# AHupuJR/REFID

Measured on AMD Instinct MI355X. Metric: interpolated frames/sec (train step) GoPro 256x256 11+1, higher is better.
Workload: dtype f32

## Files before the change

refid_amd/csrc/conv_args.h:

```cpp
#pragma once

struct ConvKArgs {
    const float* inA; const float* inB;
    int ldA, ldB, Ca, Ctot;
    const float* w; const float* bias;
    float* out; int ldO;
    const float* res; int ldR;
    const float* mask; int ldM;
    int N, H, W, Ho, Wo;
    int Cout, CoutPad, coBase;
    int pad, nchunks, tilesX, tilesY;
    float slopePre, slopePost, slopeMask;
    long long wClsStride;
    int vecOK;
    int ncot;
    int bf16;
    int ksplit = 1;
    long long wsStride = 0;
    int gridTiles = 0;
    const float* add2 = nullptr; float* out2 = nullptr; int ldA2 = 0, ldO2 = 0;
    int maskMode = 0;
    int shuffle = 0;
    int patchW = 0, patchRow = 0;
};


size_t refid_wino3x3_workspace_bytes(const ConvKArgs& a, int split_mode);
int refid_launch_wino3x3(const ConvKArgs& a, float* ws, size_t ws_bytes, int split_mode, int tile_hint, hipStream_t st);
int refid_launch_splitk_finish(const ConvKArgs& f, const float* ws, int ldW, long long npix, hipStream_t st);
bool refid_wino6_eligible(const ConvKArgs& a);
size_t refid_wino6_workspace_bytes(const ConvKArgs& a, int split_mode);
int refid_launch_wino6(const ConvKArgs& a, float* ws, size_t ws_bytes, int split_mode, int tile_hint, int terms, hipStream_t st);
bool refid_split3x3_eligible(const ConvKArgs& a);
int refid_launch_split3x3(const ConvKArgs& a, int terms, int mode, int cus, int split_mode, hipStream_t st);
struct PwExtra {
    const float* lnG = nullptr; const float* lnB = nullptr; float lnEps = 0.f; float* lnOut = nullptr; int ldLn = 0;
    const float* pool = nullptr; int poolParts = 0; float invHW = 0.f; int hw = 0; int seC = 0;
    const float* seW1 = nullptr; const float* seB1 = nullptr; const float* seW2 = nullptr; const float* seB2 = nullptr;
    float* seM = nullptr; float* seZ1 = nullptr; float* seS = nullptr;
    float* xsOut = nullptr; int ldXs = 0;
    const float* res2 = nullptr; int ldR2 = 0;
    float* out2 = nullptr; int ldO2 = 0;
};
int refid_launch_pointwise(const ConvKArgs& a, hipStream_t st, const PwExtra* ex = nullptr, int terms = 0);
```

refid_amd/csrc/conv_igemm.hip:

```cpp
#include "common.h"
#include "conv_args.h"

namespace {

template <int KH_, int KW_, int S_, int WM_, int WN_, int MT_, int NT_, int NSUB_, int MODE_>
struct Cfg {
    static constexpr int KH = KH_, KW = KW_, S = S_, WM = WM_, WN = WN_, MT = MT_, NT = NT_;
    static constexpr int NSUB = NSUB_, MODE = MODE_;
    static constexpr int TW = 32;
    static constexpr int TH = WM * MT;
    static constexpr int BN = WN * NT * 32;
    static constexpr int NTAPS = (MODE == 2) ? 4 : KH * KW;
    static constexpr int HH = (MODE == 2) ? TH + 2 : (TH - 1) * S + KH;
    static constexpr int HWD = (MODE == 2) ? TW + 2 : (TW - 1) * S + KW;
    static constexpr int HP = HH * HWD;
    static constexpr int NQ = NSUB * 2;
    static constexpr int KC = NSUB * 8;
    static constexpr int A_TOTAL = HP * NQ;
    static constexpr int B_TOTAL = NTAPS * BN * NQ;
    static constexpr int A_ITEMS = (A_TOTAL + 255) / 256;
    static constexpr int B_ITEMS = (B_TOTAL + 255) / 256;
    static constexpr int LDS_BYTES = (A_TOTAL + B_TOTAL) * 16;
    static_assert(WM * WN == 4, "4 waves per workgroup");
    static_assert(256 % NQ == 0, "thread -> channel-quad mapping must be static");
// ... 371 lines not shown
    a.Ca = d->c_a; a.Ctot = d->c_a + d->c_b;
    a.N = d->n; a.H = d->h; a.W = d->w; a.Ho = d->ho; a.Wo = d->wo;
    a.Cout = d->cout; a.CoutPad = d->cout_pad; a.coBase = d->co_base;
    a.vecOK = 1;
    if (d->algo == 1) return refid_wino3x3_workspace_bytes(a, d->split_k);
    if (d->algo == 5) return refid_wino6_workspace_bytes(a, d->split_k);
    if (d->algo != 0 && d->algo != 2) return 0;
    const bool bf = d->algo == 2;
    const int bn = refid_conv_bn(d->kh, d->kw, d->stride, d->mode, d->cout);
    switch (family_of(d->kh, d->kw, d->stride, d->mode)) {
        case F_4x4s2: return igemm_ws_bytes<C4S2_64>(a, 1, d->split_k, bf);
        case F_downDgrad: return bn == 64 ? igemm_ws_bytes<CD_64>(a, 4, d->split_k, bf) : igemm_ws_bytes<CD_128>(a, 4, d->split_k, bf);
        default: return 0;
    }
}

extern "C" int refid_conv2d(const refid_conv_desc* d, void* stream) {
    hipStream_t st = reinterpret_cast<hipStream_t>(stream);
    REFID_CHECK(d != nullptr, "conv2d: null descriptor");
    const Family f = family_of(d->kh, d->kw, d->stride, d->mode);
    REFID_CHECK(f != F_none, "conv2d: unsupported geometry k=%dx%d stride=%d mode=%d", d->kh, d->kw,
                d->stride, d->mode);
    REFID_CHECK(d->in_a && d->w_packed && d->out, "conv2d: null tensor pointer");
    REFID_CHECK(d->c_a > 0 && d->c_a % 4 == 0 && d->c_b % 4 == 0 && d->c_b >= 0,
                "conv2d: channel counts must be multiples of 4 (c_a=%d c_b=%d)", d->c_a, d->c_b);
    REFID_CHECK(d->ld_a % 4 == 0 && (d->c_b == 0 || d->ld_b % 4 == 0),
                "conv2d: pixel pitches must be multiples of 4 floats");
    REFID_CHECK(d->c_b == 0 || d->in_b != nullptr, "conv2d: c_b > 0 but in_b is null");
    REFID_CHECK(d->n > 0 && d->h > 0 && d->w > 0 && d->ho > 0 && d->wo > 0 && d->cout > 0,
                "conv2d: empty problem (n=%d h=%d w=%d ho=%d wo=%d cout=%d)", d->n, d->h, d->w, d->ho,
                d->wo, d->cout);
    REFID_CHECK(d->pw == nullptr || d->algo == 3, "conv2d: pw fusions belong to the pointwise tile (algo 3)");
    REFID_CHECK(d->algo == 0 || d->algo == 2 || ((d->algo == 1 || d->algo == 5) && f == F_3x3) || (d->algo == 3 && (f == F_1x1 || f == F_convT || f == F_2x2s2)) ||
                    (d->algo == 4 && (f == F_3x3 || f == F_4x4s2 || f == F_downDgrad)),
                "conv2d: algo %d does not fit this geometry (1 / 5 = 3x3 stride 1, 3 = 1x1 and ConvTranspose2d(2,2), 4 = 3x3 stride 1 / 4x4 stride 2 and "
                "its input gradient)", d->algo);
    REFID_CHECK(d->algo != 2 || d->c_b == 0 || d->c_a % 8 == 0, "conv2d: bf16 tile needs c_a %% 8 == 0 for two sources");
    const int bn = refid_conv_bn(d->kh, d->kw, d->stride, d->mode, d->cout);
    REFID_CHECK(d->co_base >= 0 && d->co_base + d->cout <= d->cout_pad,
                "conv2d: rows [%d, %d) exceed the packed weight's %d rows", d->co_base, d->co_base + d->cout,
                d->cout_pad);
    if (d->mode == 0) {
        const int eh = (d->h + 2 * d->pad - d->kh) / d->stride + 1;
        const int ew = (d->w + 2 * d->pad - d->kw) / d->stride + 1;
        REFID_CHECK(eh == d->ho && ew == d->wo, "conv2d: output size %dx%d does not match geometry (%dx%d)",
                    d->ho, d->wo, eh, ew);
    } else {
        REFID_CHECK(d->ho == d->h && d->wo == d->w, "conv2d: mode %d needs ho,wo == h,w", d->mode);
        REFID_CHECK(d->mode != 1 || d->cout % 4 == 0, "conv2d: mode 1 needs cout = 4*Co");
    }
    ConvKArgs a;
    a.inA = d->in_a; a.inB = d->in_b; a.ldA = d->ld_a; a.ldB = d->ld_b;
    a.Ca = d->c_a; a.Ctot = d->c_a + d->c_b;
    a.w = d->w_packed; a.bias = d->bias;
    a.out = d->out; a.ldO = d->ld_out;
    a.res = d->res; a.ldR = d->ld_res;
    a.mask = d->mask; a.ldM = d->ld_mask;
    a.add2 = d->add2; a.ldA2 = d->ld_add2; a.out2 = d->out2; a.ldO2 = d->ld_out2;
    a.maskMode = d->mask_mode;
    REFID_CHECK(d->mask_mode == 0 || (d->mask_mode == 1 && d->algo == 3 && d->mask != nullptr),
                "conv2d: mask_mode 1 (GELU derivative) belongs to the pointwise tile (algo 3) and needs a mask tensor");
    REFID_CHECK(d->out2 == nullptr || (d->add2 != nullptr && (d->algo != 3 || d->pw == nullptr)),
                "conv2d: out2 needs add2 (and, on the pointwise tile, no fusions)");
    a.N = d->n; a.H = d->h; a.W = d->w; a.Ho = d->ho; a.Wo = d->wo;
    a.Cout = d->cout; a.CoutPad = d->cout_pad; a.coBase = d->co_base;
    a.pad = d->pad; a.nchunks = 0; a.tilesX = a.tilesY = 0;
    a.slopePre = d->slope_pre; a.slopePost = d->slope_post; a.slopeMask = d->slope_mask;
    auto al16 = [](const void* p) { return (reinterpret_cast<uintptr_t>(p) & 15) == 0; };
    a.vecOK = al16(d->out) && d->ld_out % 4 == 0 && (!d->res || (al16(d->res) && d->ld_res % 4 == 0)) &&
// ... 21 lines not shown
            REFID_CHECK((long long)d->n * d->h * d->w * d->ld_a * 4 < 0x7fffffffLL, "conv2d: tensor too large for the pointwise tile's 32-bit offsets");
            return refid_launch_pointwise(a, st, nullptr, 0);
        }
        REFID_CHECK(d->c_b == 0 || d->c_a % 8 == 0, "conv2d: pointwise tile needs c_a %% 8 == 0 for two sources");
        const long long lim = 0x7fffffffLL;
        REFID_CHECK((long long)d->n * d->h * d->w * d->ld_a * 4 < lim &&
                        (d->c_b == 0 || (long long)d->n * d->h * d->w * d->ld_b * 4 < lim),
                    "conv2d: tensor too large for the pointwise tile's 32-bit offsets (use algo 0)");
        if (d->pw != nullptr) {
            const refid_pw_extras* x = d->pw;
            PwExtra e;
            e.lnG = x->ln_gamma; e.lnB = x->ln_beta; e.lnEps = x->ln_eps; e.lnOut = x->ln_out; e.ldLn = x->ld_ln_out;
            e.pool = x->pool; e.poolParts = x->pool_parts; e.invHW = x->inv_hw; e.hw = x->hw; e.seC = x->se_c;
            e.seW1 = x->se_w1; e.seB1 = x->se_b1; e.seW2 = x->se_w2; e.seB2 = x->se_b2;
            e.seM = x->se_m; e.seZ1 = x->se_z1; e.seS = x->se_s;
            e.xsOut = x->xs_out; e.ldXs = x->ld_xs_out;
            e.res2 = x->res2; e.ldR2 = x->ld_res2;
            e.out2 = x->out2; e.ldO2 = x->ld_out2;
            auto al = [](const void* q, int ld) { return (reinterpret_cast<uintptr_t>(q) & 15) == 0 && ld % 4 == 0; };
            REFID_CHECK((!e.lnOut || al(e.lnOut, e.ldLn)) && (!e.xsOut || al(e.xsOut, e.ldXs)) && (!e.res2 || al(e.res2, e.ldR2)) &&
                            (!e.out2 || al(e.out2, e.ldO2)) && (!e.lnG || (al(e.lnG, 4) && al(e.lnB, 4))),
                        "conv2d: pointwise fusion tensors must be 16-byte aligned with pitches that are multiples of 4");
            return refid_launch_pointwise(a, st, &e, d->mfma_terms);
        }
        return refid_launch_pointwise(a, st, nullptr, d->mfma_terms);
    }
    if (d->algo == 4) {
        static int cus = 0;
        if (cus == 0) cus = refid_device_cu_count();
        REFID_CHECK(d->pad == 1, "conv2d: the split tile's geometries all have pad 1");
        return refid_launch_split3x3(a, d->mfma_terms ? d->mfma_terms : 6, f == F_3x3 ? 0 : (f == F_4x4s2 ? 1 : 2),
                                     cus > 0 ? cus : 256, d->split_k, st);
    }
    if (d->algo == 5) return refid_launch_wino6(a, d->ws, d->ws_bytes, d->split_k, d->wino_tile, d->mfma_terms, st);
    if (d->algo == 1) {
        REFID_CHECK(d->c_b == 0 || d->c_a % 8 == 0, "conv2d: Winograd tile needs c_a %% 8 == 0 for two sources");
        const long long lim = 0x7fffffffLL;
        REFID_CHECK((long long)d->n * d->h * d->w * d->ld_a * 4 < lim &&
                        (d->c_b == 0 || (long long)d->n * d->h * d->w * d->ld_b * 4 < lim),
                    "conv2d: tensor too large for the Winograd tile's 32-bit offsets (use algo 0)");
        return refid_launch_wino3x3(a, d->ws, d->ws_bytes, d->split_k, d->wino_tile, st);
    }
    switch (f) {
        case F_3x3:
            if (bn == 32) return launch<C3_32>(a, 1, st);
            if (bn == 64) return launch<C3_64>(a, 1, st);
            return launch<C3_128>(a, 1, st);
        case F_5x5: return launch<C5_32>(a, 1, st);
        case F_1x1:
            if (bn == 32) return launch<C1_32>(a, 1, st);
            if (bn == 64) return launch<C1_64>(a, 1, st);
            return launch<C1_128>(a, 1, st);
        case F_4x4s2: return launch<C4S2_64>(a, 1, st, SplitArgs{d->ws, d->ws_bytes, d->split_k});
        case F_2x2s2: return bn == 64 ? launch<C2S2_64>(a, 1, st) : launch<C2S2_128>(a, 1, st);
        case F_convT: return bn == 64 ? launch<CT_64>(a, 1, st) : launch<CT_128>(a, 1, st);
        case F_downDgrad: {
            const SplitArgs sp{d->ws, d->ws_bytes, d->split_k};
            return bn == 64 ? launch<CD_64>(a, 4, st, sp) : launch<CD_128>(a, 4, st, sp);
        }
        default: break;
    }
    refid_set_error("conv2d: no tile for this geometry");
    return 1;
}
```

refid_amd/engine.py:

```python
import os
from collections import OrderedDict

import torch

from . import ops
from ._lib import RefidHipError


def param_shapes(img_chn, ev_chn=2, out_chn=3, base=32, num_residual_blocks=2, num_block=1, num_encoders=3):
    b = base
    sh = OrderedDict()

    def conv(name, co, ci, k, bias=True):
        sh[name + ".weight"] = (co, ci, k, k)
        if bias:
            sh[name + ".bias"] = (co,)

    conv("head.conv2d", b, ev_chn, 5)
    enc_in = [b * 2 ** i for i in range(num_encoders)]
    enc_out = [b * 2 ** (i + 1) for i in range(num_encoders)]

    def evr(prefix, ci, co, fuse, atten):
        conv(prefix + ".conv.conv2d", co, ci, 3)
        if atten:
# ... 100 lines not shown
def use_pipeline(b, h, w):
    return PIPELINE if isinstance(PIPELINE, bool) else b * h * w <= PIPELINE_MAX_PIX
PACK_BATCH = os.environ.get("REFID_PACK_BATCH", "1") != "0"
LAZY_FALLBACK_PACKS = os.environ.get("REFID_LAZY_PACKS", "1") != "0"
CONVT_PW = os.environ.get("REFID_CONVT_PW", "1") != "0"
CONVT_PWS = os.environ.get("REFID_CONVT_PWS", "1") != "0"
ROWS_DEFER = os.environ.get("REFID_ROWS_DEFER", "0") != "0"
FINISH_BATCH = os.environ.get("REFID_FINISH_BATCH", "1") != "0"
FUSE_SUMS = os.environ.get("REFID_FUSE_SUMS", "1") != "0"
LINEAR_SPLIT = os.environ.get("REFID_LINEAR_SPLIT", "1") != "0"


class _SideStreams:
    def __init__(self):
        self._s = {}

    def get(self, device):
        if device.type != "cuda":
            return None
        s = self._s.get(device.index)
        if s is None:
            s = self._s[device.index] = torch.cuda.Stream(device=device)
        return s


DEC_STREAM = _SideStreams()
LV_STREAMS = (_SideStreams(), _SideStreams(), _SideStreams())
WINO6 = os.environ.get("REFID_WINO6", "1") != "0"
_WF16 = os.environ.get("REFID_WINO_F16", "1")
WINO_F16_FWD = _WF16 in ("1", "fwd")
WINO_F16_DGRAD = _WF16 in ("1", "dgrad")
WINO6_MIN_CO = int(os.environ.get("REFID_WINO6_MIN_CO", "32"))
WINO6_THIN = os.environ.get("REFID_WINO6_THIN", "1") != "0"
DOWN_SPLIT = int(os.environ.get("REFID_DOWN_SPLIT", "6"))
WGRAD_WINO_MIN_CO = int(os.environ.get("REFID_WGRAD_WINO_MIN_CO", "32"))
_WG_ENV = os.environ.get("REFID_WGRAD_GROUP")
WGRAD_GROUP = max(1, min(24, int(_WG_ENV))) if _WG_ENV else 24
WGRAD_KEEP_BYTES_PER_PIXEL_STEP = 4900
PWS_WGRAD = os.environ.get("REFID_PWS_WGRAD", "1") != "0"
WGRAD_F4 = os.environ.get("REFID_WGRAD_F4", "1") != "0"
WGRAD_F4_MIN_HW = int(os.environ.get("REFID_WGRAD_F4_MIN_HW", "16"))
WGRAD_DOWN_F4 = os.environ.get("REFID_WGRAD_DOWN_F4", "1") != "0"


def wgrad_group_cap(n, pixels, device, free_bytes=None):
    if n <= 1 or pixels <= 0:
        return n
    if free_bytes is None:
        if torch.device(device).type != "cuda":
            return n
        free_bytes = torch.cuda.mem_get_info(device)[0] + (torch.cuda.memory_reserved(device) - torch.cuda.memory_allocated(device))
    per_step = pixels * WGRAD_KEEP_BYTES_PER_PIXEL_STEP
    return max(1, min(n, int(free_bytes // 2 // per_step)))


FILL_MIN_WG = int(os.environ.get("REFID_FILL_MIN_WG", "256"))


def _fills_gpu(n, ho, wo, cout, classes):
    if ops.WINO_SPLIT != 2:
        n = 8
    return n * -(-ho // 4) * -(-wo // 32) * -(-cout // 64) * classes >= FILL_MIN_WG


_LIM4 = (2 ** 31 - 1) // 4

# ... 134 lines not shown
        if wd6 is not None and wd6.nbytes() >= 2 ** 31 - 1:
            wd6 = None
        terms = 1 if bf16 else (3 if compute_dtype == "bf16x3" else 0)
        sf_pad = sd_pad = 0
        if terms and kind == "conv" and k == 3 and ci % 8 == 0 and co >= 16:
            self.split = terms
            planes = {1: 1, 3: 2}[terms]
            sf_bn = ops.conv_bn(3, 3, 1, 0, co)
            sf_pad = -(-co // sf_bn) * sf_bn
            if not (fp16 and wp6 is not None):
                wps = _Packing("wps", "split", (ops.ROLE_FWD, sf_bn, 3, 3, co, ci, planes))
            if need_dgrad and co % 8 == 0 and (not (fp16 and wd6 is not None) or (ci == 2 * co and co < WINO6_MIN_CO)):
                sd_bn = self.d_bn if self.d_algo != 1 else ops.conv_bn(3, 3, 1, 0, min(ci, 128))
                if ci == 2 * co:
                    sd_bn = ops.conv_bn(3, 3, 1, 0, co)
                sd_pad = -(-ci // sd_bn) * sd_bn
                wds = _Packing("wds", "split", (ops.ROLE_DGRAD, sd_bn, 3, 3, co, ci, planes))
        if kind == "down" and ci % 8 == 0 and co % 8 == 0 and (terms or DOWN_SPLIT):
            self.split = terms = terms or DOWN_SPLIT
            planes = {1: 1, 3: 2, 6: 3, ops.TERMS_F16X3: 2}[terms]
            f16 = terms == ops.TERMS_F16X3
            if not bf16:
                sf_bn = ops.conv_bn(4, 4, 2, 0, co)
                sf_pad = -(-co // sf_bn) * sf_bn
                wps = _Packing("wps", "split", (ops.ROLE_FWD, sf_bn, 4, 4, co, ci, planes), f16)
            if need_dgrad:
                sd_bn = ops.conv_bn(4, 4, 2, 2, ci)
                sd_pad = -(-ci // sd_bn) * sd_bn
                wds = _Packing("wds", "split", (ops.ROLE_DOWN_DGRAD, sd_bn, 4, 4, co, ci, planes), f16)
        self.wp_lazy = wp.lazy = LAZY_FALLBACK_PACKS and wp6 is not None and (self.f_algo == 1 or fp16)
        self.wd_lazy = LAZY_FALLBACK_PACKS and wd6 is not None and (self.d_algo == 1 or fp16)
        if wd is not None:
            wd.lazy = self.wd_lazy
        self.packings = [p for p in (wp, wd, wp6, wd6, wps, wds) if p is not None]
        self._lazy = {p.attr: p for p in self.packings if p.lazy}
        self.wd = self.wp6 = self.wd6 = self.wps = self.wds = None
        for p in self.packings:
            setattr(self, p.attr, p.alloc(self.w.device))
        self.b_eff = self.b
        if self.scale is not None and self.has_bias:
            self.b_eff = torch.empty_like(self.b)
        kh, kw, st, md = f_geo
        self._f_split = self._f_wino6 = self._d_split = self._d_wino6 = self._d_plain = None
        if wps is not None:
            self._f_split = ("wps", dict(kh=kh, kw=kw, stride=st, pad=1, mode=0, cout_pad=sf_pad, algo=4, terms=self.split), True, False)
        if wp6 is not None and (self.split == 0 or fp16):
            self._f_wino6 = ("wp6", dict(kh=3, kw=3, stride=1, pad=1, mode=0, cout_pad=-(-self.f_rows // 64) * 64, algo=5,
                                     terms=wp6.flag), True, False)
        self._f_plain = ("wp", dict(kh=kh, kw=kw, stride=st, pad=self.pad, mode=md, cout_pad=self.f_pad, algo=self.f_algo),
                         self.f_algo != 3, True)
        if need_dgrad:
            kh, kw, st, md = d_geo
            if wds is not None:
                self._d_split = ("wds", dict(kh=kh, kw=kw, stride=st, pad=1, mode=md, cout_pad=sd_pad, algo=4, terms=self.split), True, False)
            if wd6 is not None and (self.split == 0 or fp16):
                self._d_wino6 = ("wd6", dict(kh=3, kw=3, stride=1, pad=1, mode=0, cout_pad=-(-self.d_rows // 64) * 64, algo=5,
                                         terms=wd6.flag), True, False)
            self._d_plain = ("wd", dict(kh=kh, kw=kw, stride=st, pad=d_padding, mode=md, cout_pad=self.d_pad, algo=self.d_algo),
                             self.d_algo != 3 or kind == "convT", self.d_algo == 3 and kind == "conv")
        self.wslab = None
        self.w_calls = 0
        self.w_last = None
        self.w_pend = []
        self.w_algo, self.w_bias = 0, True
        self.w_group = 1

    def plan_repack(self, plan):
        for p in self.packings:
            if not p.lazy:
                p.plan(self, plan)
        if self.scale is not None and self.has_bias:
            plan.add_mul_vec(self.b, self.scale, self.b_eff)

    def _packed(self, attr):
        p = self._lazy.get(attr)
        if p is not None and p.epoch != self.arena.pack_epoch:
            p.pack(self)
        return getattr(self, attr)

    def pack_fallbacks(self):
        for attr in self._lazy:
            self._packed(attr)

    def repack(self):
        for p in self.packings:
            p.pack(self)
        if self.scale is not None and self.has_bias:
            ops.mul_vec(self.b, self.scale, out=self.b_eff)

    def _fwd_route(self, n, ho, wo, a, b, pw):
        r = self._f_split
        if r is not None and (self.split > 1 or b is None) and a.shape[3] % 8 == 0 and pw is None and \
                (self.kind == "conv" or (b is None and _fills_gpu(n, ho, wo, self.co, 1))):
            return r
        r = self._f_wino6
        if r is not None and (b is None or a.shape[3] % 16 == 0):
            return r
        return self._f_plain

    def fwd(self, a, b=None, res=None, slope_pre=1.0, slope_post=1.0, out=None, pw=None, bias=True, plus=None):
        n, h, w, _ = a.shape
        bv = self.b_eff if bias else None
        if self.kind == "conv":
            ho, wo, oc = h, w, self.co
        elif self.kind == "down":
            ho, wo, oc = h // 2, w // 2, self.co
        else:
            ho, wo, oc = 2 * h, 2 * w, self.co
        if out is None:
            out = torch.empty((n, ho, wo, _pad4(oc)), dtype=torch.float32, device=a.device)
            if _pad4(oc) != oc:
                out.zero_()
                out = out[..., :oc]
        o2 = torch.empty_like(out) if plus is not None else None
        parts = ((a, b, res, out),)
        if n * a.stride(0) >= _LIM4 or n * out.stride(0) >= _LIM4 or (b is not None and n * b.stride(0) >= _LIM4):
            if pw is not None:
                raise RefidHipError(f"{self.name}: fused pointwise extras cannot be issued in sub-batches (tensor >= 2 GiB)")
            parts = _sub_batches(n, a, b, res, out)
        for a_i, b_i, res_i, out_i in parts:
            attr, geo, fused, takes_pw = self._fwd_route(a_i.shape[0], ho, wo, a_i, b_i, pw)
            fused = fused and plus is not None and len(parts) == 1
            extra = dict(add2=plus, out2=o2) if fused else {}
            if takes_pw:
                extra["pw"] = pw
            ops.conv2d(a_i, self._packed(attr), out_i, cout=self.f_rows, in_b=b_i, bias=bv, res=res_i, slope_pre=slope_pre,
                       slope_post=slope_post, **geo, **extra)
        if plus is None:
            return out
        if not fused:
            ops.add(out, plus, out=o2)
        return out, o2

    def can_fwd_from(self):
        return self.kind == "conv" and self.k == 1 and self.f_algo == 3 and not self.bf16

    def fwd_from(self, a, k_base):
        if not self.can_fwd_from() or k_base % self.f_kc or a.shape[3] % self.f_kc:
            raise RefidHipError(f"{self.name}: fwd_from needs the fp32 pointwise tile and chunk-aligned channel blocks")
        n, h, w, _ = a.shape
        out = torch.empty((n, h, w, self.co), dtype=torch.float32, device=a.device)
        ops.conv2d(a, self.wp[(k_base // self.f_kc) * self.f_pad * self.f_kc:], out, kh=1, kw=1, stride=1, pad=0, mode=0,
                   cout=self.f_rows, cout_pad=self.f_pad, bias=self.b_eff, algo=3)
        return out

    def _dgrad_route(self, g, cnt):
        r = self._d_wino6
        if self.fp16 and r is not None and cnt >= WINO6_MIN_CO:
            return r
        r = self._d_split
        if r is not None and (self.kind == "conv" or _fills_gpu(g.shape[0], g.shape[1], g.shape[2], cnt, 4)):
            return r
        r = self._d_wino6
        if r is not None and cnt >= WINO6_MIN_CO:
            return r
        return self._d_plain

    def gelu_mask_ok(self, g, rows=None):
        return self.wd is not None and self._dgrad_route(g, rows[1] if rows is not None else self.d_rows)[3]

    def dgrad(self, g, rows=None, res=None, mask=None, slope_mask=1.0, out=None, plus=None, gelu_mask=False):
        if self.wd is None:
            raise RefidHipError(f"{self.name}: dgrad weights were not requested")
        base, cnt = rows if rows is not None else (0, self.d_rows)
        n, h, w, _ = g.shape
        if self.kind == "conv":
            ho, wo = h, w
        elif self.kind == "down":
            ho, wo = 2 * h, 2 * w
        else:
            ho, wo = h // 2, w // 2
        if out is None:
            out = torch.empty((n, ho, wo, cnt), dtype=torch.float32, device=g.device)
        o2 = torch.empty_like(out) if plus is not None else None
        parts = ((g, res, mask, out),)
        if n * g.stride(0) >= _LIM4 or n * out.stride(0) >= _LIM4:
            parts = _sub_batches(n, g, res, mask, out)
        for g_i, res_i, mask_i, out_i in parts:
            attr, geo, fused, gelu_ok = self._dgrad_route(g_i, cnt)
# ... 710 lines not shown
                    if g_Sb[i] is None:
                        g_Sb[i] = L.fuse.dgrad(g_f, rows=(C, C))
                    else:
                        L.fuse.dgrad(g_f, rows=(C, C), res=g_Sb[i], out=g_Sb[i])
                g_s = L.fuse.dgrad(g_f, rows=(0, C), res=g_hf[i])
                g_o = self._evr_first_bwd(L, g_s, st, g_hf, g_xb, g_e, t, B, c["ip_f"], g_skip, True, keep if lin else None)

        if lin:
            self.pred.wgrad(g4sum, head, bias=False)
            g_xb[NL - 1] = ops.sum_n(keep["gb0"])
            for i, L in enumerate(self.enc_f):
                gsum = ops.sum_n(keep["gf"][i])
                if L.zero_s is None:
                    L.fuse.wgrad(gsum, Sb[i], bias=False, i_base=L.C)
                else:
                    L.fuse.wgrad(gsum, L.zero_s, Sb[i], bias=False)
                g_Sb[i] = L.fuse.dgrad(gsum, rows=(L.C, L.C))
            for i in range(2, NL):
                self._lin_level2_tail(self.enc_f[i], keep["gu"][i], xb, g_xb, first=g_xb[i - 1] is None)
            g_xb[0] = ops.sum_n(keep["gy"])
        self._egaca_img_bwd(self.enc_f[1].att, xb[0], g_xb[0], c["ip_f"])
        finish_wgrads(self.early_ops)
        self._egaca_fold_back(self.enc_f[1].att)
        return dict(c=c, B=B, g_xb=g_xb, g_Sb=g_Sb, g_e=g_e, g_head=g_head)

    def backward_late(self, state):
        c, B, g_xb, g_Sb, g_e, g_head = (state[k] for k in ("c", "B", "g_xb", "g_Sb", "g_e", "g_head"))
        xb, head, e_all = c["xb"], c["head"], c["e_all"]
        if ROWS_DEFER:
            ops.rows_sum_defer()
        NL = self.NL
        g_hb = [None] * NL
        lin = c["lin"]
        keep = dict(gy=[], gu={i: [] for i in range(2, NL)})
        for t, sts in reversed(c["steps_b"]):
            g_o = None
            for i in range(NL - 1, -1, -1):
                L, st = self.enc_b[i], sts[i]
                carry = g_hb[i] if g_hb[i] is not None else g_Sb[i]
                if i == NL - 1:
                    g_s = carry
                else:
                    L.down.wgrad(g_o, st["s"])
                    g_s = L.down.dgrad(g_o, res=carry)
                g_o = self._evr_first_bwd(L, g_s, st, g_hb, g_xb, g_e, t, B, c["ip_b"], None, False, keep if lin else None)
        if lin:
            for i in range(2, NL):
                self._lin_level2_tail(self.enc_b[i], keep["gu"][i], xb, g_xb, first=False)
            ops.sum_n([g_xb[0]] + keep["gy"], out=g_xb[0])

        self._egaca_img_bwd(self.enc_b[1].att, xb[0], g_xb[0], c["ip_b"])
        gz_e = ops.act_bwd(g_e, e_all, 0.2, out=g_e)
        self.head_ev.wgrad(gz_e, c["ev_in"])
        g = g_xb[NL - 1]
        for i in range(NL - 1, -1, -1):
            E = self.img[i]
            gin, c1, c2, sm = c["img_saved"][i]
            E["down"].wgrad(g, sm)
            g_sm = E["down"].dgrad(g)
            E["identity"].wgrad(g_sm, gin)
            gz2 = ops.act_bwd(g_sm, c2, 0.2)
            E["conv_2"].wgrad(gz2, c1)
            g_c1 = E["conv_2"].dgrad(gz2, mask=c1, slope_mask=0.2)
            E["conv_1"].wgrad(g_c1, gin)
            acc = g_xb[i - 1] if i > 0 else g_head
            t1 = E["identity"].dgrad(g_sm, res=acc)
            if i > 0:
                g = E["conv_1"].dgrad(g_c1, res=t1)
            else:
                g = E["conv_1"].dgrad(g_c1, res=t1, mask=head, slope_mask=0.2)
        self.head_img.wgrad(g, c["x_in"])
        finish_wgrads(self.all_ops)
        self._egaca_fold_back(self.enc_b[1].att)

    def _lin_level2_tail(self, L, gu, xb, g_xb, first):
        k = L.level - 1
        gsum = ops.sum_n(gu)
        L.conv.wgrad(gsum, xb[k], bias=False)
        if first:
            g_xb[k] = L.conv.dgrad(gsum)
        else:
            L.conv.dgrad(gsum, res=g_xb[k], out=g_xb[k])

    def _evr_first_bwd(self, L, g_s, st, g_h, g_xb, g_e, t, B, ip, g_skip, first_writer, keep=None):
        i = L.level
        lin = keep is not None
        if i == 1:
            g_u, g_h[i] = self._trunk_bwd(L.trunk, g_s, st)
            g_in = self._egaca_bwd(L.att, g_u, None if lin else g_xb[0], ip, st, keep["gy"] if lin else None)
            if g_skip is not None:
                g_in = ops.add(g_in, g_skip[0], out=g_in)
            return g_in
        g_u, g_h[i] = self._trunk_bwd(L.trunk, g_s, st, mask_u=st["u"], slope_u=0.04)
        L.conv.wgrad(g_u, st["src"])
        if i >= 2:
            if lin:
                keep["gu"][i].append(g_u)
                return L.conv.dgrad(g_u, res=g_skip[i - 1] if g_skip is not None else None)
            g_a2 = L.conv.dgrad(g_u)
            ops.add(g_xb[i - 1], g_a2, out=g_xb[i - 1])
            if g_skip is not None:
                g_a2 = ops.add(g_a2, g_skip[i - 1], out=g_a2)
            return g_a2
        sl = g_e[t * B:(t + 1) * B]
        if first_writer:
            L.conv.dgrad(g_u, out=sl)
        else:
            L.conv.dgrad(g_u, res=sl, out=sl)
        return None
```

refid_amd/ops.py:

```python
import ctypes as C
import os

import torch

from . import _lib
from ._lib import ConvDesc, WgradDesc, check, lib

ROLE_FWD, ROLE_DGRAD, ROLE_CONVT, ROLE_CONVT_DGRAD, ROLE_DOWN_DGRAD, ROLE_WINO_FWD, ROLE_WINO_DGRAD, ROLE_CONVT_DGRAD_PW = range(8)


WINO_SPLIT = {"0": 0, "s": 1}.get(os.environ.get("REFID_SPLITK", os.environ.get("REFID_WINO_SPLITK", "auto"))[:1], 2)

WINO_TILE = int(os.environ.get("REFID_WINO_TILE", "0"))

PROFILE = None


def _stream():
    return C.c_void_p(torch.cuda.current_stream().cuda_stream)


_REQUIRE_CUDA = True


# ... 204 lines not shown
    d.slope_pre, d.slope_post, d.slope_mask = slope_pre, slope_post, slope_mask
    d.mask_mode = mask_mode
    d.algo = algo
    d.wino_tile = WINO_TILE
    if WINO_SPLIT and algo in (0, 1, 2, 4, 5):
        d.split_k = WINO_SPLIT
        need = lib().refid_conv_workspace_bytes(C.byref(d))
        if need:
            ws = _workspace(need, in_a.device, "conv")
            d.ws, d.ws_bytes = ws.data_ptr(), ws.numel() * 4
    if PROFILE is None:
        check(lib().refid_conv2d(C.byref(d), _stream()), "refid_conv2d")
        return out
    e0, e1 = torch.cuda.Event(enable_timing=True), torch.cuda.Event(enable_timing=True)
    e0.record()
    check(lib().refid_conv2d(C.byref(d), _stream()), "refid_conv2d")
    e1.record()
    taps = {0: kh * kw, 1: 1, 2: 16}[mode]
    flops = 2.0 * d.n * d.ho * d.wo * cout * (d.c_a + d.c_b) * taps
    name = "conv_igemm_kernel<" + lib().refid_conv_tile_name(kh, kw, stride, mode, cout).decode() + \
        (", true> [bf16 operands]" if algo == 2 else ">")
    if algo == 1:
        name = "conv_wino_kernel<1, 2>" if cout <= 32 else "conv_wino_kernel<2, 1>"
    if algo == 5:
        name = "conv_wino6_kernel<2>" if cout > 32 else "conv_wino6_kernel<1>"
        if terms == 3:
            name = name[:-1] + ", true>"
        if terms == 1:
            name = name[:-1] + ", true, fp16x1>"
    if algo == 4:
        name = "conv_split_kernel<%s>" % ("3, fp16" if terms == TERMS_F16X3 else (terms or 6))
    if algo == 3:
        name = "conv_pw_kernel<1, 8>" if cout <= 32 else ("conv_pw_kernel<2, 4, six>" if terms == 6 else "conv_pw_kernel<2, 4>")
    opix = d.n * out.shape[1] * out.shape[2]
    nbytes = 4.0 * (d.n * d.h * d.w * (d.c_a + d.c_b) + opix * out.shape[3] * (1 + (res is not None) + (mask is not None))
                    + cout * (d.c_a + d.c_b) * taps)
    if out2 is not None:
        nbytes += 8.0 * opix * out.shape[3]
    if pw is not None:
        for k in ("ln_out", "xs_out", "out2", "res2"):
            if pw.get(k) is not None:
                nbytes += 4.0 * pw[k].numel()
    PROFILE.append((name, flops, e0, e1,
                    (d.n, d.h, d.w, d.c_a, d.c_b, cout, int(res is not None), int(mask is not None), int(bias is not None)),
                    nbytes))
    return out


DESC_CACHE = os.environ.get("REFID_DESC_CACHE", "0") == "1"
_DESC_CACHE = {}
_DESC_PTRS = ("in_a", "in_b", "w_packed", "bias", "out", "res", "mask", "add2", "out2")


def _sig(t):
    return None if t is None else (t.shape, t.stride())


def _conv2d_cached(in_a, w_packed, out, kh, kw, stride, pad, mode, cout, cout_pad, co_base, in_b, bias, res, mask,
                   slope_pre, slope_post, slope_mask, algo, terms, add2, out2, mask_mode):
    global lib, DESC_CACHE
    key = (kh, kw, stride, pad, mode, cout, cout_pad, co_base, slope_pre, slope_post, slope_mask, algo, terms, mask_mode,
           WINO_TILE, WINO_SPLIT, _sig(in_a), _sig(in_b), _sig(out), _sig(res), _sig(mask), _sig(add2), _sig(out2),
           bias is not None, in_a.dtype, out.dtype, in_a.device)
    ent = _DESC_CACHE.get(key)
    if ent is None:
        real, seen = lib(), []
# ... 593 lines not shown
```

Before: 515.3.

## Add thin-channel conv kernels for input and output ends, fold head mask into dgrad

Adds a persistent, double-buffered MFMA kernel for convolutions with 4 stored input channels (3x3/5x5), with weights held in registers and halos staged in LDS as channel planes. Also adds an optional direct-FMA kernel for at most 4 output channels, and folds the head's leaky-ReLU backward mask into the last dgrad epilogue so a separate act_bwd pass is skipped. These target the first and last layers, which the generic implicit-GEMM tile wastes work on because it pads channels to 8 or 32. The thin-input forward route and the mask fold are on by default; the dgrad and prediction routes are behind environment flags.

New measurement: 518.4 (median of 6 runs). About the same (+0.6%).

```diff
diff --git a/refid_amd/csrc/conv_args.h b/refid_amd/csrc/conv_args.h
--- a/refid_amd/csrc/conv_args.h
+++ b/refid_amd/csrc/conv_args.h
@@ -43,3 +43,5 @@
     float* out2 = nullptr; int ldO2 = 0;
 };
 int refid_launch_pointwise(const ConvKArgs& a, hipStream_t st, const PwExtra* ex = nullptr, int terms = 0);
+int refid_launch_thin_in(const ConvKArgs& a, int kh, int kw, int stride, int mode, int pairs, hipStream_t st);
+int refid_launch_thin_out(const ConvKArgs& a, int kh, int kw, int stride, int mode, hipStream_t st);
diff --git a/refid_amd/csrc/conv_igemm.hip b/refid_amd/csrc/conv_igemm.hip
--- a/refid_amd/csrc/conv_igemm.hip
+++ b/refid_amd/csrc/conv_igemm.hip
@@ -427,9 +427,10 @@
                 d->wo, d->cout);
     REFID_CHECK(d->pw == nullptr || d->algo == 3, "conv2d: pw fusions belong to the pointwise tile (algo 3)");
     REFID_CHECK(d->algo == 0 || d->algo == 2 || ((d->algo == 1 || d->algo == 5) && f == F_3x3) || (d->algo == 3 && (f == F_1x1 || f == F_convT || f == F_2x2s2)) ||
-                    (d->algo == 4 && (f == F_3x3 || f == F_4x4s2 || f == F_downDgrad)),
-                "conv2d: algo %d does not fit this geometry (1 / 5 = 3x3 stride 1, 3 = 1x1 and ConvTranspose2d(2,2), 4 = 3x3 stride 1 / 4x4 stride 2 and "
-                "its input gradient)", d->algo);
+                    (d->algo == 4 && (f == F_3x3 || f == F_4x4s2 || f == F_downDgrad)) || (d->algo == 6 && (f == F_3x3 || f == F_5x5)) ||
+                    (d->algo == 7 && f == F_3x3),
+                "conv2d: algo %d does not fit this geometry (1 / 5 / 7 = 3x3 stride 1, 3 = 1x1 and ConvTranspose2d(2,2), 4 = 3x3 stride 1 / 4x4 stride 2 and "
+                "its input gradient, 6 = 3x3 / 5x5 stride 1)", d->algo);
     REFID_CHECK(d->algo != 2 || d->c_b == 0 || d->c_a % 8 == 0, "conv2d: bf16 tile needs c_a %% 8 == 0 for two sources");
     const int bn = refid_conv_bn(d->kh, d->kw, d->stride, d->mode, d->cout);
     REFID_CHECK(d->co_base >= 0 && d->co_base + d->cout <= d->cout_pad,
@@ -517,6 +518,8 @@
         return refid_launch_split3x3(a, d->mfma_terms ? d->mfma_terms : 6, f == F_3x3 ? 0 : (f == F_4x4s2 ? 1 : 2),
                                      cus > 0 ? cus : 256, d->split_k, st);
     }
+    if (d->algo == 6) return refid_launch_thin_in(a, d->kh, d->kw, d->stride, d->mode, d->mfma_terms, st);
+    if (d->algo == 7) return refid_launch_thin_out(a, d->kh, d->kw, d->stride, d->mode, st);
     if (d->algo == 5) return refid_launch_wino6(a, d->ws, d->ws_bytes, d->split_k, d->wino_tile, d->mfma_terms, st);
     if (d->algo == 1) {
         REFID_CHECK(d->c_b == 0 || d->c_a % 8 == 0, "conv2d: Winograd tile needs c_a %% 8 == 0 for two sources");
diff --git a/refid_amd/csrc/conv_thin.hip b/refid_amd/csrc/conv_thin.hip
--- /dev/null
+++ b/refid_amd/csrc/conv_thin.hip
@@ -0,0 +1,288 @@
+#include "common.h"
+#include "conv_args.h"
+
+namespace {
+
+__device__ __forceinline__ void thin_epilogue(const ConvKArgs& a, f32x4 v, int j0, long long op, bool vec) {
+    const int ch = j0;
+    f32x4 bv = {0.f, 0.f, 0.f, 0.f};
+    if (a.bias) {
+        const float* bp = a.bias + a.coBase + j0;
+        if (vec) bv = *reinterpret_cast<const f32x4*>(bp);
+        else
+#pragma unroll
+            for (int k = 0; k < 4; ++k) if (j0 + k < a.Cout) bv[k] = bp[k];
+    }
+#pragma unroll
+    for (int k = 0; k < 4; ++k) v[k] = lrelu(v[k] + bv[k], a.slopePre);
+    if (vec) {
+        if (a.res) v += *reinterpret_cast<const f32x4*>(a.res + op * a.ldR + ch);
+#pragma unroll
+        for (int k = 0; k < 4; ++k) v[k] = lrelu(v[k], a.slopePost);
+        if (a.mask) {
+            const f32x4 mv = *reinterpret_cast<const f32x4*>(a.mask + op * a.ldM + ch);
+#pragma unroll
+            for (int k = 0; k < 4; ++k) v[k] *= (mv[k] > 0.f) ? 1.f : a.slopeMask;
+        }
+        *reinterpret_cast<f32x4*>(a.out + op * a.ldO + ch) = v;
+        if (a.out2)
+            *reinterpret_cast<f32x4*>(a.out2 + op * a.ldO2 + ch) = v + *reinterpret_cast<const f32x4*>(a.add2 + op * a.ldA2 + ch);
+    } else {
+#pragma unroll
+        for (int k = 0; k < 4; ++k) {
+            if (j0 + k >= a.Cout) break;
+            float t = v[k];
+            if (a.res) t += a.res[op * a.ldR + ch + k];
+            t = lrelu(t, a.slopePost);
+            if (a.mask) t *= (a.mask[op * a.ldM + ch + k] > 0.f) ? 1.f : a.slopeMask;
+            a.out[op * a.ldO + ch + k] = t;
+            if (a.out2) a.out2[op * a.ldO2 + ch + k] = t + a.add2[op * a.ldA2 + ch + k];
+        }
+    }
+}
+
+template <int K, int NP>
+struct ThinIn {
+    static constexpr int TH = 4, TW = 32;
+    static constexpr int HH = TH + K - 1, HWD = TW + K - 1, HP = HH * HWD;
+    static constexpr int PLANE = HP + ((32 - HP % 64) + 64) % 64;
+    static constexpr int NCH = 2 * NP;
+    static constexpr int ITEMS = (HP + 255) / 256;
+    static constexpr int BUF = NCH * PLANE;
+};
+
+template <int K, int NP>
+__global__ __launch_bounds__(256) void conv_thin_in_kernel(const ConvKArgs a) {
+    using C = ThinIn<K, NP>;
+    __shared__ float sX[2 * C::BUF];
+
+    const int tid = threadIdx.x;
+    const int lane = tid & 63, wave = tid >> 6;
+    const int li = lane & 31, kh = lane >> 5;
+
+    float wr[K * K][NP];
+    {
+        const bool rowOK = li < a.Cout && a.coBase + li < a.CoutPad;
+#pragma unroll
+        for (int t = 0; t < K * K; ++t)
+#pragma unroll
+            for (int p = 0; p < NP; ++p)
+                wr[t][p] = rowOK ? a.w[((long long)t * a.CoutPad + a.coBase + li) * 8 + 2 * p + kh] : 0.f;
+    }
+
+    const float bv = (a.bias && li < a.Cout) ? a.bias[a.coBase + li] : 0.f;
+
+    const int tilesPerImg = a.tilesX * a.tilesY;
+    const int ntiles = tilesPerImg * a.N;
+    f32x4 ra[C::ITEMS];
+
+    auto load_halo = [&](int tile) {
+        const int n = tile / tilesPerImg;
+        const int r = tile - n * tilesPerImg;
+        const int ty = r / a.tilesX, tx = r - ty * a.tilesX;
+        const int iy0 = ty * C::TH - a.pad, ix0 = tx * C::TW - a.pad;
+#pragma unroll
+        for (int it = 0; it < C::ITEMS; ++it) {
+            const int hp = tid + it * 256;
+            const int hy = hp / C::HWD, hx = hp - hy * C::HWD;
+            const int iy = iy0 + hy, ix = ix0 + hx;
+            f32x4 v = {0.f, 0.f, 0.f, 0.f};
+            if (hp < C::HP && iy >= 0 && iy < a.H && ix >= 0 && ix < a.W)
+                v = *reinterpret_cast<const f32x4*>(a.inA + ((long long)(n * a.H + iy) * a.W + ix) * a.ldA);
+            ra[it] = v;
+        }
+    };
+    auto store_halo = [&](float* buf) {
+#pragma unroll
+        for (int it = 0; it < C::ITEMS; ++it) {
+            const int hp = tid + it * 256;
+            if (hp < C::HP) {
+#pragma unroll
+                for (int c = 0; c < C::NCH; ++c) buf[c * C::PLANE + hp] = ra[it][c];
+            }
+        }
+    };
+
+    int tile = blockIdx.x;
+    if (tile >= ntiles) return;
+    load_halo(tile);
+    store_halo(sX);
+    __syncthreads();
+
+    int cur = 0;
+    for (; tile < ntiles; tile += gridDim.x) {
+        const int next = tile + gridDim.x;
+        const bool more = next < ntiles;
+        if (more) load_halo(next);
+
+        const float* pX = sX + cur * C::BUF + kh * C::PLANE + wave * C::HWD + li;
+        f32x16 acc;
+#pragma unroll
+        for (int r = 0; r < 16; ++r) acc[r] = 0.f;
+#pragma unroll
+        for (int t = 0; t < K * K; ++t) {
+            const int toff = (t / K) * C::HWD + (t % K);
+#pragma unroll
+            for (int p = 0; p < NP; ++p)
+                acc = __builtin_amdgcn_mfma_f32_32x32x2f32(pX[2 * p * C::PLANE + toff], wr[t][p], acc, 0, 0, 0);
+        }
+
+        const int n = tile / tilesPerImg;
+        const int rt = tile - n * tilesPerImg;
+        const int ty = rt / a.tilesX, tx = rt - ty * a.tilesX;
+        const int oy = ty * C::TH + wave;
+        if (oy < a.Ho && li < a.Cout) {
+            const long long op0 = (long long)(n * a.Ho + oy) * a.Wo + tx * C::TW;
+            const int wleft = a.Wo - tx * C::TW;
+#pragma unroll
+            for (int r = 0; r < 16; ++r) {
+                const int px = 8 * (r >> 2) + 4 * kh + (r & 3);
+                if (px >= wleft) continue;
+                const long long op = op0 + px;
+                float t = lrelu(acc[r] + bv, a.slopePre);
+                if (a.res) t += a.res[op * a.ldR + li];
+                t = lrelu(t, a.slopePost);
+                if (a.mask) t *= (a.mask[op * a.ldM + li] > 0.f) ? 1.f : a.slopeMask;
+                a.out[op * a.ldO + li] = t;
+                if (a.out2) a.out2[op * a.ldO2 + li] = t + a.add2[op * a.ldA2 + li];
+            }
+        }
+
+        if (more) store_halo(sX + (cur ^ 1) * C::BUF);
+        __syncthreads();
+        cur ^= 1;
+    }
+}
+
+template <int K, int NP>
+int launch_thin_in(const ConvKArgs& ka, int cus, hipStream_t st) {
+    using C = ThinIn<K, NP>;
+    ConvKArgs a = ka;
+    a.tilesX = cdiv(a.Wo, C::TW);
+    a.tilesY = cdiv(a.Ho, C::TH);
+    const long long ntiles = (long long)a.tilesX * a.tilesY * a.N;
+    REFID_CHECK(ntiles < 0x7fffffffLL, "conv2d: too many output tiles for the thin-input tile (algo 6)");
+    long long walk = (ntiles + 16LL * cus - 1) / (16LL * cus);
+    if (walk < 2) walk = 2;
+    const int grid = (int)((ntiles + walk - 1) / walk);
+    hipLaunchKernelGGL((conv_thin_in_kernel<K, NP>), dim3(grid), dim3(256), 0, st, a);
+    REFID_LAUNCH_CHECK("conv_thin_in");
+    return 0;
+}
+
+struct ThinOut {
+    static constexpr int TH = 4, TW = 32, NT = TH * TW;
+    static constexpr int HH = TH + 2, HWD = TW + 2, HP = HH * HWD;
+    static constexpr int NQ = 8;
+    static constexpr int ITEMS = (HP * NQ + NT - 1) / NT;
+};
+
+template <int NCO>
+__global__ __launch_bounds__(ThinOut::NT) void conv_thin_out_kernel(const ConvKArgs a) {
+    using C = ThinOut;
+    __shared__ f32x4 sX[C::NQ * C::HP];
+
+    const int tid = threadIdx.x;
+    int bt = blockIdx.x;
+    const int tx = bt % a.tilesX; bt /= a.tilesX;
+    const int ty = bt % a.tilesY;
+    const int n = bt / a.tilesY;
+    const int iy0 = ty * C::TH - 1, ix0 = tx * C::TW - 1;
+    const int nq = a.Ctot >> 2;
+
+    f32x4 ra[C::ITEMS];
+#pragma unroll
+    for (int it = 0; it < C::ITEMS; ++it) {
+        const int e = tid + it * C::NT;
+        const int q = e % C::NQ, hp = e / C::NQ;
+        const int hy = hp / C::HWD, hx = hp - hy * C::HWD;
+        const int iy = iy0 + hy, ix = ix0 + hx;
+        f32x4 v = {0.f, 0.f, 0.f, 0.f};
+        if (hp < C::HP && q < nq && iy >= 0 && iy < a.H && ix >= 0 && ix < a.W)
+            v = *reinterpret_cast<const f32x4*>(a.inA + ((long long)(n * a.H + iy) * a.W + ix) * a.ldA + 4 * q);
+        ra[it] = v;
+    }
+#pragma unroll
+    for (int it = 0; it < C::ITEMS; ++it) {
+        const int e = tid + it * C::NT;
+        const int q = e % C::NQ, hp = e / C::NQ;
+        if (hp < C::HP) sX[q * C::HP + hp] = ra[it];
+    }
+    __syncthreads();
+
+    const int py = tid >> 5, px = tid & 31;
+    float acc[NCO];
+#pragma unroll
+    for (int co = 0; co < NCO; ++co) acc[co] = 0.f;
+    const float* wrow = a.w + (long long)a.coBase * 8;
+    const int tapStride = a.CoutPad * 8;
+    for (int q = 0; q < nq; ++q) {
+        const float* wq = wrow + (long long)(q >> 1) * 9 * tapStride + (q & 1) * 4;
+        const f32x4* xq = sX + q * C::HP + py * C::HWD + px;
+#pragma unroll
+        for (int t = 0; t < 9; ++t) {
+            const f32x4 x = xq[(t / 3) * C::HWD + (t % 3)];
+#pragma unroll
+            for (int co = 0; co < NCO; ++co) {
+                const f32x4 w = *reinterpret_cast<const f32x4*>(wq + t * tapStride + co * 8);
+#pragma unroll
+                for (int k = 0; k < 4; ++k) acc[co] = __builtin_fmaf(x[k], w[k], acc[co]);
+            }
+        }
+    }
+
+    const int oy = ty * C::TH + py, ox = tx * C::TW + px;
+    if (oy < a.Ho && ox < a.Wo) {
+        const long long op = (long long)(n * a.Ho + oy) * a.Wo + ox;
+        f32x4 v = {0.f, 0.f, 0.f, 0.f};
+#pragma unroll
+        for (int co = 0; co < NCO; ++co) v[co] = acc[co];
+        thin_epilogue(a, v, 0, op, a.vecOK && a.Cout == 4);
+    }
+}
+
+template <int NCO>
+int launch_thin_out(const ConvKArgs& ka, hipStream_t st) {
+    using C = ThinOut;
+    ConvKArgs a = ka;
+    a.tilesX = cdiv(a.Wo, C::TW);
+    a.tilesY = cdiv(a.Ho, C::TH);
+    const long long ntiles = (long long)a.tilesX * a.tilesY * a.N;
+    REFID_CHECK(ntiles < 0x7fffffffLL, "conv2d: too many output tiles for the thin-output tile (algo 7)");
+    hipLaunchKernelGGL((conv_thin_out_kernel<NCO>), dim3((int)ntiles), dim3(C::NT), 0, st, a);
+    REFID_LAUNCH_CHECK("conv_thin_out");
+    return 0;
+}
+
+}
+
+int refid_launch_thin_in(const ConvKArgs& a, int kh, int kw, int stride, int mode, int pairs, hipStream_t st) {
+    REFID_CHECK(stride == 1 && mode == 0, "conv2d: the thin-input tile (algo 6) is stride 1, mode 0 (stride=%d mode=%d)", stride, mode);
+    REFID_CHECK(kh == kw && (kh == 3 || kh == 5), "conv2d: the thin-input tile (algo 6) is 3x3 or 5x5 (kh=%d kw=%d)", kh, kw);
+    REFID_CHECK(a.Ca == 4 && a.Ctot == 4, "conv2d: the thin-input tile (algo 6) takes one source of c_a = 4 stored input channels "
+                "(c_a=%d c_b=%d)", a.Ca, a.Ctot - a.Ca);
+    REFID_CHECK(a.Cout <= 32, "conv2d: the thin-input tile (algo 6) writes at most 32 output channels (cout=%d)", a.Cout);
+    REFID_CHECK(pairs == 0 || pairs == 1 || pairs == 2, "conv2d: algo 6 takes mfma_terms = 1 (input channels 0-1 only) or 0 / 2 (all four), "
+                "got mfma_terms=%d", pairs);
+    REFID_CHECK(a.pad >= 0 && a.pad < kh, "conv2d: the thin-input tile (algo 6) needs 0 <= pad < k (pad=%d)", a.pad);
+    static int cus = 0;
+    if (cus == 0) cus = refid_device_cu_count();
+    const int c = cus > 0 ? cus : 256;
+    if (kh == 5) return pairs == 1 ? launch_thin_in<5, 1>(a, c, st) : launch_thin_in<5, 2>(a, c, st);
+    return pairs == 1 ? launch_thin_in<3, 1>(a, c, st) : launch_thin_in<3, 2>(a, c, st);
+}
+
+int refid_launch_thin_out(const ConvKArgs& a, int kh, int kw, int stride, int mode, hipStream_t st) {
+    REFID_CHECK(stride == 1 && mode == 0, "conv2d: the thin-output tile (algo 7) is stride 1, mode 0 (stride=%d mode=%d)", stride, mode);
+    REFID_CHECK(kh == 3 && kw == 3 && a.pad == 1, "conv2d: the thin-output tile (algo 7) is 3x3 with pad 1 (kh=%d kw=%d pad=%d)", kh, kw, a.pad);
+    REFID_CHECK(a.Ca == a.Ctot && a.Ctot <= 32, "conv2d: the thin-output tile (algo 7) takes one source of at most 32 input channels "
+                "(c_a=%d c_b=%d)", a.Ca, a.Ctot - a.Ca);
+    REFID_CHECK(a.Cout <= 4, "conv2d: the thin-output tile (algo 7) writes at most 4 output channels (cout=%d)", a.Cout);
+    REFID_CHECK((reinterpret_cast<uintptr_t>(a.w) & 15) == 0, "conv2d: the thin-output tile (algo 7) needs a 16-byte aligned w_packed");
+    switch (a.Cout) {
+        case 1: return launch_thin_out<1>(a, st);
+        case 2: return launch_thin_out<2>(a, st);
+        case 3: return launch_thin_out<3>(a, st);
+        default: return launch_thin_out<4>(a, st);
+    }
+}
diff --git a/refid_amd/engine.py b/refid_amd/engine.py
--- a/refid_amd/engine.py
+++ b/refid_amd/engine.py
@@ -156,6 +156,15 @@
 WINO_F16_DGRAD = _WF16 in ("1", "dgrad")
 WINO6_MIN_CO = int(os.environ.get("REFID_WINO6_MIN_CO", "32"))
 WINO6_THIN = os.environ.get("REFID_WINO6_THIN", "1") != "0"
+
+
+def thin_ends_mode():
+    return int(os.environ.get("REFID_THIN_ENDS", "1"))
+
+
+THIN_DGRAD = os.environ.get("REFID_THIN_DGRAD", "0") != "0"
+THIN_PRED_FWD = os.environ.get("REFID_THIN_PRED_FWD", "0") != "0"
+HEAD_MASK_FOLD = os.environ.get("REFID_HEAD_MASK_FOLD", "1") != "0"
 DOWN_SPLIT = int(os.environ.get("REFID_DOWN_SPLIT", "6"))
 WGRAD_WINO_MIN_CO = int(os.environ.get("REFID_WGRAD_WINO_MIN_CO", "32"))
 _WG_ENV = os.environ.get("REFID_WGRAD_GROUP")
@@ -356,9 +365,16 @@
         self.wd_lazy = LAZY_FALLBACK_PACKS and wd6 is not None and (self.d_algo == 1 or fp16)
         if wd is not None:
             wd.lazy = self.wd_lazy
-        self.packings = [p for p in (wp, wd, wp6, wd6, wps, wds) if p is not None]
+        thin = not bf16 and kind == "conv"
+        thin_f_in = thin and k in (3, 5) and _pad4(ci) == 4 and co <= 32 and self.f_algo == 0 and self.f_kc == 8 and self.f_bn == 32
+        thin_f_out = THIN_PRED_FWD and thin and k == 3 and co <= 4 and ci <= 32 and ci % 4 == 0 and self.f_algo == 0 and self.f_kc == 8
+        thin_d_in = THIN_DGRAD and thin and need_dgrad and k in (3, 5) and _pad4(co) == 4 and ci <= 32
+        wdt = None
+        if thin_d_in and not (self.d_algo == 0 and self.d_kc == 8 and self.d_bn == 32):
+            wdt = _Packing("wdt", "pack", (ops.ROLE_DGRAD, 32, 8, k, k, co, ci), False)
+        self.packings = [p for p in (wp, wd, wp6, wd6, wps, wds, wdt) if p is not None]
         self._lazy = {p.attr: p for p in self.packings if p.lazy}
-        self.wd = self.wp6 = self.wd6 = self.wps = self.wds = None
+        self.wd = self.wp6 = self.wd6 = self.wps = self.wds = self.wdt = None
         for p in self.packings:
             setattr(self, p.attr, p.alloc(self.w.device))
         self.b_eff = self.b
@@ -373,6 +389,16 @@
                                      terms=wp6.flag), True, False)
         self._f_plain = ("wp", dict(kh=kh, kw=kw, stride=st, pad=self.pad, mode=md, cout_pad=self.f_pad, algo=self.f_algo),
                          self.f_algo != 3, True)
+        self._f_thin = self._d_thin = None
+        if thin_f_in:
+            self._f_thin = ("wp", dict(kh=k, kw=k, stride=1, pad=self.pad, mode=0, cout_pad=self.f_pad, algo=6,
+                                       terms=1 if ci <= 2 else 2), True, False)
+        elif thin_f_out:
+            self._f_thin = ("wp", dict(kh=3, kw=3, stride=1, pad=1, mode=0, cout_pad=self.f_pad, algo=7), True, False)
+        self._thin_ca = 4 if thin_f_in else ci
+        if thin_d_in:
+            self._d_thin = ("wdt" if wdt is not None else "wd",
+                            dict(kh=k, kw=k, stride=1, pad=d_padding, mode=0, cout_pad=32, algo=6, terms=1 if co <= 2 else 2), True, False)
         if need_dgrad:
             kh, kw, st, md = d_geo
             if wds is not None:
@@ -413,6 +439,15 @@
             ops.mul_vec(self.b, self.scale, out=self.b_eff)
 
     def _fwd_route(self, n, ho, wo, a, b, pw):
+        r = self._f_thin
+        if r is not None:
+            mode = thin_ends_mode()
+            if mode and b is None and pw is None and a.shape[3] == self._thin_ca:
+                return r
+            if mode == 2:
+                raise RefidHipError(f"{self.name}: REFID_THIN_ENDS=2, but this forward call cannot take the streaming kernel "
+                                    f"(one source of {self._thin_ca} stored channels, no pointwise fusions; got "
+                                    f"{a.shape[3]} channels{', a second source' if b is not None else ''})")
         r = self._f_split
         if r is not None and (self.split > 1 or b is None) and a.shape[3] % 8 == 0 and pw is None and \
                 (self.kind == "conv" or (b is None and _fills_gpu(n, ho, wo, self.co, 1))):
@@ -469,6 +504,14 @@
         return out
 
     def _dgrad_route(self, g, cnt):
+        r = self._d_thin
+        if r is not None:
+            mode = thin_ends_mode()
+            if mode and g.shape[3] == 4:
+                return r
+            if mode == 2:
+                raise RefidHipError(f"{self.name}: REFID_THIN_ENDS=2, but this input-gradient call cannot take the streaming kernel "
+                                    f"(4 stored gradient channels; got {g.shape[3]})")
         r = self._d_wino6
         if self.fp16 and r is not None and cnt >= WINO6_MIN_CO:
             return r
@@ -1245,6 +1288,7 @@
         NL = self.NL
         g_hb = [None] * NL
         lin = c["lin"]
+        fold = HEAD_MASK_FOLD and thin_ends_mode() != 0 and len(c["steps_b"]) == c["T"]
         keep = dict(gy=[], gu={i: [] for i in range(2, NL)})
         for t, sts in reversed(c["steps_b"]):
             g_o = None
@@ -1256,14 +1300,15 @@
                 else:
                     L.down.wgrad(g_o, st["s"])
                     g_s = L.down.dgrad(g_o, res=carry)
-                g_o = self._evr_first_bwd(L, g_s, st, g_hb, g_xb, g_e, t, B, c["ip_b"], None, False, keep if lin else None)
+                g_o = self._evr_first_bwd(L, g_s, st, g_hb, g_xb, g_e, t, B, c["ip_b"], None, False, keep if lin else None,
+                                          e_mask=e_all if fold else None)
         if lin:
             for i in range(2, NL):
                 self._lin_level2_tail(self.enc_b[i], keep["gu"][i], xb, g_xb, first=False)
             ops.sum_n([g_xb[0]] + keep["gy"], out=g_xb[0])
 
         self._egaca_img_bwd(self.enc_b[1].att, xb[0], g_xb[0], c["ip_b"])
-        gz_e = ops.act_bwd(g_e, e_all, 0.2, out=g_e)
+        gz_e = g_e if fold else ops.act_bwd(g_e, e_all, 0.2, out=g_e)
         self.head_ev.wgrad(gz_e, c["ev_in"])
         g = g_xb[NL - 1]
         for i in range(NL - 1, -1, -1):
@@ -1295,7 +1340,7 @@
         else:
             L.conv.dgrad(gsum, res=g_xb[k], out=g_xb[k])
 
-    def _evr_first_bwd(self, L, g_s, st, g_h, g_xb, g_e, t, B, ip, g_skip, first_writer, keep=None):
+    def _evr_first_bwd(self, L, g_s, st, g_h, g_xb, g_e, t, B, ip, g_skip, first_writer, keep=None, e_mask=None):
         i = L.level
         lin = keep is not None
         if i == 1:
@@ -1318,6 +1363,8 @@
         sl = g_e[t * B:(t + 1) * B]
         if first_writer:
             L.conv.dgrad(g_u, out=sl)
+        elif e_mask is not None:
+            L.conv.dgrad(g_u, res=sl, out=sl, mask=e_mask[t * B:(t + 1) * B], slope_mask=0.2)
         else:
             L.conv.dgrad(g_u, res=sl, out=sl)
         return None
diff --git a/refid_amd/ops.py b/refid_amd/ops.py
--- a/refid_amd/ops.py
+++ b/refid_amd/ops.py
@@ -260,6 +260,10 @@
         name = "conv_split_kernel<%s>" % ("3, fp16" if terms == TERMS_F16X3 else (terms or 6))
     if algo == 3:
         name = "conv_pw_kernel<1, 8>" if cout <= 32 else ("conv_pw_kernel<2, 4, six>" if terms == 6 else "conv_pw_kernel<2, 4>")
+    if algo == 6:
+        name = "conv_thin_in_kernel<%d, %d>" % (kh, 1 if terms == 1 else 2)
+    if algo == 7:
+        name = "conv_thin_out_kernel<%d>" % cout
     opix = d.n * out.shape[1] * out.shape[2]
     nbytes = 4.0 * (d.n * d.h * d.w * (d.c_a + d.c_b) + opix * out.shape[3] * (1 + (res is not None) + (mask is not None))
                     + cout * (d.c_a + d.c_b) * taps)
```
